# Arash-san/YinYang-Game-AlphaZero

Measured on AMD Instinct MI355X. Metric: self-play positions/sec (+ MCTS node-expansions/sec) at 800 sims, 8x8 board, higher is better.
Workload: dtype f16x3; 1 GPU; 8x8 board, 800 sims/move, 4096 concurrent games per GPU, frozen random-init 128x10 net (seed 0), copied boards, reference_quirks=False, staggered start plies; tree_arithmetic=f32 PUCT + u64 bitboards, nn_dtype=f16x3, evaluation_reuse=False, parallelism=episode-sharded x1, lanes_per_gpu=2, hipgraph=True

## Files before the change

include/yy_engine.h:

```cpp
#ifndef YY_ENGINE_H
#define YY_ENGINE_H

#include <stdint.h>

#ifdef __cplusplus
extern "C" {
#endif

#define YY_OK 0
#define YY_E_INVALID (-1)
#define YY_E_UNSUPPORTED (-2)
#define YY_E_NOMEM (-3)
#define YY_E_HIP (-4)
#define YY_E_STATE (-5)
#define YY_E_ARENA (-6)

#define YY_FLAG_ROWCOL 1u
#define YY_FLAG_ALIASED 2u
#define YY_FLAG_REUSE_PASS_VALUE 4u

#define YY_FLAG_REUSE_TRANSPOSITIONS 8u
#define YY_FLAG_KEEP_EVALUATIONS 16u

typedef void *yy_stream_t;

const char *yy_last_error(void);
int yy_version(void);


int yy_rules_valid_mask(const int8_t *boards, const int8_t *players, int G, int R, int C,
                        uint32_t flags, uint8_t *out_mask, yy_stream_t stream);

int yy_rules_step(int8_t *boards, int8_t *players, const int32_t *actions, int G, int R, int C,
                  uint32_t flags, uint8_t *placed, yy_stream_t stream);

int yy_rules_game_ended(const int8_t *boards, const int8_t *players, int G, int R, int C,
                        uint32_t flags, double *out, int32_t *counts, yy_stream_t stream);

int yy_encode_planes(const int8_t *boards, int G, int R, int C, float *out, yy_stream_t stream);

int yy_rules_mask_terminal_bb(const uint64_t *black, const uint64_t *white, int G, int R, int C,
                              uint32_t flags, uint64_t *mask_p1, uint64_t *mask_m1,
                              int8_t *result, yy_stream_t stream);

int yy_pack_boards(const int8_t *boards, int G, int R, int C, uint64_t *black, uint64_t *white,
                   yy_stream_t stream);
int yy_unpack_boards(const uint64_t *black, const uint64_t *white, int G, int R, int C,
                     int8_t *boards, yy_stream_t stream);


typedef struct yy_mcts_config {
    int32_t G;
    int32_t R, C;
    int32_t max_sims;
    float cpuct;
    uint32_t flags;
    int64_t edges_per_game;
    int64_t nodes_per_game;
} yy_mcts_config;

typedef struct yy_mcts yy_mcts;

int yy_mcts_create(const yy_mcts_config *cfg, yy_mcts **out);
int yy_mcts_destroy(yy_mcts *ctx);
int yy_mcts_memory_bytes(const yy_mcts *ctx, uint64_t *out);

int yy_mcts_begin(yy_mcts *ctx, const int8_t *boards, const int8_t *root_players,
                  const uint8_t *active, float *planes_out, yy_stream_t stream);

int yy_mcts_expand_root(yy_mcts *ctx, const float *policy, const double *noise, double eps,
                        yy_stream_t stream);

int yy_mcts_select(yy_mcts *ctx, float *planes_out, uint8_t *needs_eval, yy_stream_t stream);

int yy_mcts_expand_backup(yy_mcts *ctx, const float *policy, const float *value,
                          yy_stream_t stream);

int yy_mcts_step(yy_mcts *ctx, const float *policy, const float *value, float *planes_out,
                 uint8_t *needs_eval, yy_stream_t stream);

int yy_mcts_root_counts(yy_mcts *ctx, int32_t *counts, float *child_w, float *child_p,
                        yy_stream_t stream);

int yy_mcts_root_policy(yy_mcts *ctx, int temperature_is_zero, double *pi, yy_stream_t stream);

int yy_mcts_root_stats(yy_mcts *ctx, int32_t *visits, double *value_sum, yy_stream_t stream);

int yy_mcts_get_boards(yy_mcts *ctx, int8_t *boards, yy_stream_t stream);

int yy_mcts_status(yy_mcts *ctx, int32_t *n_overflow, uint64_t *counters);
int yy_mcts_reset_counters(yy_mcts *ctx, yy_stream_t stream);
int yy_book_insert(const uint64_t *keys, int n, int R, int C, uint32_t *meta, uint64_t *table_keys, int64_t cap,
                   int32_t *slot_of, yy_stream_t stream);
int yy_mcts_set_book(yy_mcts *ctx, const uint32_t *meta, const uint64_t *keys, const float *value, const float *policy,
                     int64_t cap, int max_stones);
int yy_mcts_cache_clear(yy_mcts *ctx, yy_stream_t stream);

int yy_nn_bias_act_bf16(void *x, const float *bias, const void *residual, int64_t rows, int C,
                        int relu, yy_stream_t stream);

int yy_nn_tower_bf16(const float *planes, const void *weights, const float *bias, void *out, int G,
                     int R, int C, int channels, int n_layers, yy_stream_t stream);

int yy_nn_tower_heads_bf16(const float *planes, const void *weights, const float *bias,
                           void *out_heads, int G, int R, int C, int channels, int n_layers,
                           yy_stream_t stream);

int yy_nn_tower_f32(const float *planes, const void *weights, const float *bias, float *out, int G,
                    int R, int C, int channels, int n_layers, yy_stream_t stream);

int yy_nn_head_finish_bf16(const void *h, int G, int A, int H, const float *w2, const float *b2,
                           float *policy, float *value, yy_stream_t stream);

int yy_nn_tower_f16x3_regs(const float *planes, const void *weights, const void *head_w, const float *bias,
                           float *out, float *out_heads, const int32_t *rows, const int32_t *n_rows, int G,
                           int R, int C, int channels, int n_layers, int weight_exp, int head_exp,
                           int act_exp, yy_stream_t stream);

int yy_nn_tower_g(const float *planes, const void *weights, const void *head_w, const float *bias, const float *head_bias,
                  float *out, float *out_heads, const int32_t *rows, const int32_t *n_rows, int G, int R, int C,
                  int channels, int n_layers, int weight_exp, int head_exp, int act_exp, int nb, int boards, int gate_lo,
                  int gate_hi, yy_stream_t stream);
int yy_nn_tower_g_forms(int channels, int *nb_out);

int yy_nn_fc_heads_f16x3(const float *feats, const void *wpk, const float *bias, const int32_t *jobs, int n_jobs,
                         float *logits, float *hidden, const int32_t *n_rows, int G, int K, int A, int H,
                         int weight_exp, int act_exp, yy_stream_t stream);

int yy_nn_head_finish_f32(const float *logits, const float *hidden, int G, int A, int H, const float *w2,
                          const float *b2, const int32_t *rows, const int32_t *n_rows, float *policy,
                          float *value, yy_stream_t stream);

int yy_compact_rows(const uint8_t *flags, int G, int32_t *rows, int32_t *n, yy_stream_t stream);

int yy_selfplay_root_noise(uint64_t seed, const int64_t *game_id, const int32_t *ply, const uint8_t *draw,
                           const uint8_t *mask, int G, int A, double alpha, double *noise, yy_stream_t stream);

int yy_selfplay_sample_actions(uint64_t seed, const int64_t *game_id, const int32_t *ply,
                               const uint8_t *searching, const double *pi, const uint8_t *mask, int G, int A,
                               int temperature_threshold, int32_t *action, yy_stream_t stream);

#ifdef __cplusplus
}
#endif
#endif
```

yinyang-game-alphazero_amd/_lib.py:

```python
import ctypes as C
import os
import subprocess

_HERE = os.path.dirname(os.path.abspath(__file__))
CSRC = os.path.join(_HERE, "csrc")
SO = os.path.join(CSRC, "libyy_hip.so")
HEADER = os.path.normpath(os.path.join(_HERE, "..", "include", "yy_engine.h"))

YY_OK = 0
YY_E_ARENA = -6
FLAG_ROWCOL = 1
FLAG_ALIASED = 2
FLAG_REUSE_PASS_VALUE = 4
FLAG_REUSE_TRANSPOSITIONS = 8
FLAG_KEEP_EVALUATIONS = 16

HIPCC_FLAGS = ["--offload-arch=gfx950", "-O3", "-std=c++17", "-fPIC", "-shared",
               "-ffp-contract=off", "-fno-fast-math", "-Wall", "-Wno-unused-function"]


class YYError(RuntimeError):
    def __init__(self, code, msg):
        super().__init__(f"libyy_hip: status {code}: {msg}")
        self.code = code


class MctsConfig(C.Structure):
    _fields_ = [("G", C.c_int32), ("R", C.c_int32), ("C", C.c_int32), ("max_sims", C.c_int32),
                ("cpuct", C.c_float), ("flags", C.c_uint32), ("edges_per_game", C.c_int64),
                ("nodes_per_game", C.c_int64)]


def build(force=False, verbose=False):
    srcs = [os.path.join(CSRC, f) for f in ("yy_engine.hip", "yy_tower.hip", "yy_towerq.hip", "yy_tower_f32.hip", "yy_tower_h3r.hip",
                                            "yy_tower_g.hip", "yy_fc_heads.hip", "yy_selfplay.hip", "yy_bitboard.h")] + [HEADER]
    if not force and os.path.exists(SO) and all(os.path.getmtime(SO) >= os.path.getmtime(s) for s in srcs):
        return SO
    hipcc = os.environ.get("HIPCC", "/opt/rocm/bin/hipcc")
    tmp = f"{SO}.{os.getpid()}.tmp"
    cmd = [hipcc] + HIPCC_FLAGS + ["-o", tmp] + [s for s in srcs if s.endswith(".hip")]
    if verbose:
        print(" ".join(cmd).replace(tmp, SO))
    try:
        subprocess.check_call(cmd)
        os.replace(tmp, SO)
    finally:
        if os.path.exists(tmp):
            os.remove(tmp)
    return SO


_LIB = None
_vp = C.c_void_p
_SIGS = {
    "yy_rules_valid_mask": [_vp, _vp, C.c_int, C.c_int, C.c_int, C.c_uint32, _vp, _vp],
    "yy_rules_step": [_vp, _vp, _vp, C.c_int, C.c_int, C.c_int, C.c_uint32, _vp, _vp],
    "yy_rules_game_ended": [_vp, _vp, C.c_int, C.c_int, C.c_int, C.c_uint32, _vp, _vp, _vp],
    "yy_encode_planes": [_vp, C.c_int, C.c_int, C.c_int, _vp, _vp],
    "yy_rules_mask_terminal_bb": [_vp, _vp, C.c_int, C.c_int, C.c_int, C.c_uint32, _vp, _vp, _vp, _vp],
    "yy_pack_boards": [_vp, C.c_int, C.c_int, C.c_int, _vp, _vp, _vp],
    "yy_unpack_boards": [_vp, _vp, C.c_int, C.c_int, C.c_int, _vp, _vp],
    "yy_mcts_create": [C.POINTER(MctsConfig), C.POINTER(_vp)],
    "yy_mcts_destroy": [_vp],
    "yy_mcts_memory_bytes": [_vp, C.POINTER(C.c_uint64)],
    "yy_mcts_begin": [_vp, _vp, _vp, _vp, _vp, _vp],
    "yy_mcts_expand_root": [_vp, _vp, _vp, C.c_double, _vp],
    "yy_mcts_select": [_vp, _vp, _vp, _vp],
    "yy_mcts_expand_backup": [_vp, _vp, _vp, _vp],
    "yy_mcts_step": [_vp, _vp, _vp, _vp, _vp, _vp],
    "yy_mcts_root_counts": [_vp, _vp, _vp, _vp, _vp],
    "yy_mcts_root_policy": [_vp, C.c_int, _vp, _vp],
    "yy_mcts_root_stats": [_vp, _vp, _vp, _vp],
    "yy_mcts_get_boards": [_vp, _vp, _vp],
    "yy_mcts_status": [_vp, C.POINTER(C.c_int32), C.POINTER(C.c_uint64)],
    "yy_mcts_reset_counters": [_vp, _vp],
    "yy_mcts_cache_clear": [_vp, _vp],
    "yy_book_insert": [_vp, C.c_int, C.c_int, C.c_int, _vp, _vp, C.c_int64, _vp, _vp],
    "yy_mcts_set_book": [_vp, _vp, _vp, _vp, _vp, C.c_int64, C.c_int],
    "yy_nn_bias_act_bf16": [_vp, _vp, _vp, C.c_int64, C.c_int, C.c_int, _vp],
    "yy_nn_tower_bf16": [_vp, _vp, _vp, _vp, C.c_int, C.c_int, C.c_int, C.c_int, C.c_int, _vp],
    "yy_nn_tower_heads_bf16": [_vp, _vp, _vp, _vp, C.c_int, C.c_int, C.c_int, C.c_int, C.c_int, _vp],
    "yy_nn_head_finish_bf16": [_vp, C.c_int, C.c_int, C.c_int, _vp, _vp, _vp, _vp, _vp],
    "yy_nn_tower_f32": [_vp, _vp, _vp, _vp, C.c_int, C.c_int, C.c_int, C.c_int, C.c_int, _vp],
    "yy_nn_head_finish_f32": [_vp, _vp, C.c_int, C.c_int, C.c_int, _vp, _vp, _vp, _vp, _vp, _vp, _vp],
    "yy_compact_rows": [_vp, C.c_int, _vp, _vp, _vp],
    "yy_nn_tower_f16x3_regs": [_vp, _vp, _vp, _vp, _vp, _vp, _vp, _vp, C.c_int, C.c_int, C.c_int, C.c_int, C.c_int, C.c_int, C.c_int,
                               C.c_int, _vp],
    "yy_nn_tower_g_forms": [C.c_int, C.POINTER(C.c_int)],
    "yy_nn_tower_g": [_vp, _vp, _vp, _vp, _vp, _vp, _vp, _vp, _vp, C.c_int, C.c_int, C.c_int, C.c_int, C.c_int, C.c_int, C.c_int,
                      C.c_int, C.c_int, C.c_int, C.c_int, C.c_int, _vp],
    "yy_nn_fc_heads_f16x3": [_vp, _vp, _vp, _vp, C.c_int, _vp, _vp, _vp, C.c_int, C.c_int, C.c_int, C.c_int, C.c_int, C.c_int, _vp],
    "yy_selfplay_root_noise": [C.c_uint64, _vp, _vp, _vp, _vp, C.c_int, C.c_int, C.c_double, _vp, _vp],
    "yy_selfplay_sample_actions": [C.c_uint64, _vp, _vp, _vp, _vp, _vp, C.c_int, C.c_int, C.c_int, _vp, _vp],
    "yy_version": [],
}


def exported_symbols():
    return sorted(list(_SIGS) + ["yy_last_error"])


def lib():
    global _LIB
    if _LIB is None:
        if not os.path.exists(SO):
            raise YYError(-100, f"{SO} is missing: run __graft_entry__.build() (hipcc --offload-arch=gfx950); "
                                "there is no CPU fallback for the product path")
        L = C.CDLL(SO)
        for name, args in _SIGS.items():
            fn = getattr(L, name)
            fn.argtypes = args
            fn.restype = C.c_int
        L.yy_last_error.restype = C.c_char_p
        L.yy_last_error.argtypes = []
        _LIB = L
    return _LIB


def check(status):
    if status != YY_OK:
        raise YYError(status, lib().yy_last_error().decode())
    return status
```

yinyang-game-alphazero_amd/csrc/yy_tower_g.hip:

```cpp
#include <hip/hip_runtime.h>
#include <math.h>
#include <stdint.h>

#include <type_traits>

#include "../../include/yy_engine.h"

typedef __attribute__((ext_vector_type(8))) _Float16 f16x8;
typedef __attribute__((ext_vector_type(2))) _Float16 f16x2;
typedef __attribute__((ext_vector_type(4))) float f32x4;
typedef __attribute__((ext_vector_type(2))) float f32x2;
typedef __attribute__((ext_vector_type(4))) unsigned int u32x4;
typedef __attribute__((ext_vector_type(2))) unsigned int u32x2;

extern "C" int yy_tower_set_err(int code, const char *msg);

namespace tg {

__device__ __forceinline__ float relu_keep_nan(float v) { return __builtin_isnan(v) ? v : fmaxf(v, 0.0f); }

template <int NW_, int NB_, int D_> struct Geo {
    static constexpr int NW = NW_, NB = NB_, D = D_, CH = 32 * NW_, NCOL = 16 * NB_;
    static constexpr int RS = (NW_ >= 3) ? 288 : 160;
    static constexpr int ZERO_OFF = NCOL * RS;
    static constexpr int PART_BYTES = ZERO_OFF + 512;
    static constexpr int RES_OFF = 2 * PART_BYTES;
    static constexpr int LDS_BYTES = RES_OFF + NW_ * 2 * NB_ * 1024;
    static constexpr int CHUNK_BYTES = NW_ * 4096;
    static_assert(9 % D_ == 0, "ring position = tap % D");
    static_assert(ZERO_OFF % 256 == 0 && PART_BYTES % 256 == 0, "zero rows / parts keep the bank phase");
    static_assert(PART_BYTES + 256 < 65536 && LDS_BYTES <= 163840, "LDS layout");
};

__device__ __forceinline__ void split_pair(const f32x2 a, uint32_t &hi, uint32_t &lo) {
    const f16x2 h = __builtin_convertvector(a, f16x2);
    const f32x2 r = a - __builtin_convertvector(h, f32x2);
    const f16x2 l = __builtin_convertvector(r, f16x2);
    hi = __builtin_bit_cast(uint32_t, h);
    lo = __builtin_bit_cast(uint32_t, l);
}
__device__ __forceinline__ f32x2 join_pair(const uint32_t hi, const uint32_t lo) {
    const f32x2 h = __builtin_convertvector(__builtin_bit_cast(f16x2, hi), f32x2);
    const f32x2 l = __builtin_convertvector(__builtin_bit_cast(f16x2, lo), f32x2);
    return h + l;
}

struct WChunk {
    f16x8 h[2], l[2];
};
__device__ __forceinline__ void load_w(WChunk &w, const unsigned char *wbase, uint32_t voff) {
    const u32x4 *p = (const u32x4 *)(wbase + voff);
    w.h[0] = __builtin_bit_cast(f16x8, p[0]);
    w.l[0] = __builtin_bit_cast(f16x8, p[64]);
    w.h[1] = __builtin_bit_cast(f16x8, p[128]);
    w.l[1] = __builtin_bit_cast(f16x8, p[192]);
}

template <class GEO> struct LaneGeo {
    uint32_t rowbase[GEO::NB], okmask[GEO::NB];
};
template <class GEO> __device__ __forceinline__ void make_lane_geo(LaneGeo<GEO> &g, int lane, int R, int C, int n_valid_cols) {
    const int n = lane & 15, kg = lane >> 4, cells = R * C;
#pragma unroll
    for (int nb = 0; nb < GEO::NB; nb++) {
        const int col = nb * 16 + n;
        const int cell = col % cells;
        const int y = cell / C, x = cell - y * C;
        g.rowbase[nb] = (uint32_t)(col * GEO::RS + kg * 16);
        uint32_t m = 0;
#pragma unroll
        for (int tap = 0; tap < 9; tap++) {
            const int sy = y + tap / 3 - 1, sx = x + tap % 3 - 1;
            if (((unsigned)sy < (unsigned)R) && ((unsigned)sx < (unsigned)C)) m |= 1u << tap;
        }
        g.okmask[nb] = (col < n_valid_cols) ? m : 0u;
    }
}
template <class GEO, int TAP>
__device__ __forceinline__ uint32_t tap_addr(int nb, int crs, const LaneGeo<GEO> &g) {
    const int shift = (TAP / 3 - 1) * crs + (TAP % 3 - 1) * GEO::RS;
    const uint32_t a = g.rowbase[nb] + (uint32_t)shift;
    return (g.okmask[nb] & (1u << TAP)) ? a : ((a & 255u) | (uint32_t)GEO::ZERO_OFF);
}

template <int NB> struct XWin {
    static constexpr int P = NB;
    f16x8 h[P], l[P];
};
template <class GEO> __device__ __forceinline__ void load_x1(XWin<GEO::NB> &f, int slot, const unsigned char *lds, uint32_t cb) {
    f.h[slot] = __builtin_bit_cast(f16x8, *(const u32x4 *)(lds + cb));
    f.l[slot] = __builtin_bit_cast(f16x8, *(const u32x4 *)(lds + cb + GEO::PART_BYTES));
}
template <bool ZERO>
__device__ __forceinline__ void mma6(f32x4 (&acc1)[2], f32x4 (&acc2)[2], const WChunk &w, const f16x8 xh, const f16x8 xl) {
    const f32x4 z = {0.f, 0.f, 0.f, 0.f};
#pragma unroll
    for (int mb = 0; mb < 2; mb++) {
        const f32x4 a = __builtin_amdgcn_mfma_f32_16x16x32_f16(w.l[mb], xh, ZERO ? z : acc2[mb], 0, 0, 0);
        acc1[mb] = __builtin_amdgcn_mfma_f32_16x16x32_f16(w.h[mb], xh, ZERO ? z : acc1[mb], 0, 0, 0);
        acc2[mb] = __builtin_amdgcn_mfma_f32_16x16x32_f16(w.h[mb], xl, a, 0, 0, 0);
    }
}

template <class GEO, int J, bool ZERO>
__device__ __forceinline__ void run_chunk(f32x4 (&acc1)[GEO::NB][2], f32x4 (&acc2)[GEO::NB][2], const WChunk &w, XWin<GEO::NB> &X,
                                          const unsigned char *lds_cur, const unsigned char *lds_next, int crs, const LaneGeo<GEO> &geo) {
    constexpr int NB = GEO::NB, P = XWin<NB>::P;
#pragma unroll
    for (int nb = 0; nb < NB; nb++) {
        mma6<ZERO>(acc1[nb], acc2[nb], w, X.h[nb % P], X.l[nb % P]);
        if (nb + P < NB) load_x1<GEO>(X, nb % P, lds_cur, tap_addr<GEO, J>(nb + P, crs, geo));
        else load_x1<GEO>(X, nb % P, lds_next, tap_addr<GEO, (J + 1) % 9>(nb + P - NB, crs, geo));
        __builtin_amdgcn_sched_group_barrier(0x008, 6, 0);
        __builtin_amdgcn_sched_group_barrier(0x100, 2, 0);
    }
}

template <class GEO, bool STEM>
__device__ __forceinline__ void run_layer(f32x4 (&acc1)[GEO::NB][2], f32x4 (&acc2)[GEO::NB][2], WChunk (&W)[GEO::D], const unsigned char *lds,
                                          const unsigned char *weights, uint32_t voff, int &chunk, int n_tower, int crs,
                                          const LaneGeo<GEO> &geo) {
    constexpr int KQ = STEM ? 1 : GEO::NW, NB = GEO::NB, D = GEO::D, P = XWin<NB>::P;
    XWin<NB> X;
#pragma unroll
    for (int nb = 0; nb < P; nb++) load_x1<GEO>(X, nb, lds, tap_addr<GEO, 0>(nb, crs, geo));
    auto step = [&](auto jt, auto zt, const unsigned char *lds_cur, const unsigned char *lds_next) {
        constexpr int J = decltype(jt)::value, S = J % D;
        run_chunk<GEO, J, decltype(zt)::value>(acc1, acc2, W[S], X, lds_cur, lds_next, crs, geo);
        load_w(W[S], weights + (size_t)min(chunk + D, n_tower - 1) * GEO::CHUNK_BYTES, voff);
        __builtin_amdgcn_sched_group_barrier(0x020, 4, 0);
        __builtin_amdgcn_sched_barrier(0);
        chunk++;
    };
    auto taps = [&](auto zt, const unsigned char *cur, const unsigned char *nxt) {
        step(std::integral_constant<int, 0>{}, zt, cur, cur);
        step(std::integral_constant<int, 1>{}, std::false_type{}, cur, cur);
        step(std::integral_constant<int, 2>{}, std::false_type{}, cur, cur);
        step(std::integral_constant<int, 3>{}, std::false_type{}, cur, cur);
        step(std::integral_constant<int, 4>{}, std::false_type{}, cur, cur);
        step(std::integral_constant<int, 5>{}, std::false_type{}, cur, cur);
        step(std::integral_constant<int, 6>{}, std::false_type{}, cur, cur);
        step(std::integral_constant<int, 7>{}, std::false_type{}, cur, cur);
        step(std::integral_constant<int, 8>{}, std::false_type{}, cur, nxt);
    };
    taps(std::true_type{}, lds, lds + 64);
#pragma unroll 1
    for (int kq = 1; kq < KQ; kq++) taps(std::false_type{}, lds + kq * 64, lds + (kq + 1) * 64);
}

template <int NW_, int NB_, int D_>
__global__ void __launch_bounds__(64 * NW_, 1)
k_tower_g(const float *__restrict__ planes, const unsigned char *__restrict__ weights, const unsigned char *__restrict__ head_w,
          const float *__restrict__ bias, const float *__restrict__ head_bias, float *__restrict__ out, float *__restrict__ out_heads,
          const int *__restrict__ rows, const int *__restrict__ n_rows, int G, int R, int C, int TB, int n_layers, float in_scale,
          float acc_scale, float head_scale, float out_scale, int gate_lo, int gate_hi) {
    using GEO = Geo<NW_, NB_, D_>;
    constexpr int NW = GEO::NW, NB = GEO::NB, D = GEO::D, CH = GEO::CH, RS = GEO::RS, NT = 64 * NW_;
    __shared__ __attribute__((aligned(256))) unsigned char lds[GEO::LDS_BYTES];
    const int n_live = n_rows ? min(*n_rows, G) : G;
    if (n_live <= gate_lo || n_live > gate_hi) return;
    const int g0 = blockIdx.x * TB;
    if (g0 >= n_live) return;
    const int lane = threadIdx.x & 63;
    const int wave = __builtin_amdgcn_readfirstlane(threadIdx.x >> 6);
    const int cells = R * C, ncol = TB * cells;
    const int n_tower = 9 + 9 * NW * (n_layers - 1), crs = C * RS;

    const uint32_t voff = (uint32_t)(wave * 4096 + lane * 16);
    WChunk W[D];
#pragma unroll
    for (int j = 0; j < D; j++) load_w(W[j], weights + (size_t)min(j, n_tower - 1) * GEO::CHUNK_BYTES, voff);

    for (int t = threadIdx.x; t < 128; t += NT)
        ((u32x2 *)(lds + GEO::ZERO_OFF + (t >> 6) * GEO::PART_BYTES))[t & 63] = (u32x2){0u, 0u};
    for (int col = threadIdx.x; col < GEO::NCOL; col += NT) {
        const int gb = g0 + col / cells, cell = col % cells;
        const bool live = col < ncol && gb < n_live;
        const int src = live ? (rows ? rows[gb] : gb) : 0;
        float p[6];
#pragma unroll
        for (int k = 0; k < 5; k++) p[k] = live ? planes[((size_t)src * 5 + k) * cells + cell] * in_scale : 0.0f;
        p[5] = 0.0f;
        uint32_t hi[3], lo[3];
#pragma unroll
        for (int k = 0; k < 3; k++) split_pair((f32x2){p[2 * k], p[2 * k + 1]}, hi[k], lo[k]);
        const u32x4 z = {0u, 0u, 0u, 0u};
        *(u32x4 *)(lds + col * RS) = (u32x4){hi[0], hi[1], hi[2], 0u};
        *(u32x4 *)(lds + GEO::PART_BYTES + col * RS) = (u32x4){lo[0], lo[1], lo[2], 0u};
#pragma unroll
        for (int q = 1; q < 4; q++) {
            *(u32x4 *)(lds + col * RS + 16 * q) = z;
            *(u32x4 *)(lds + GEO::PART_BYTES + col * RS + 16 * q) = z;
        }
    }

    LaneGeo<GEO> geo;
    make_lane_geo<GEO>(geo, lane, R, C, ncol);
    const int n16 = lane & 15, kg = lane >> 4;
    unsigned char *res_lds = lds + GEO::RES_OFF + (wave * 2 * NB) * 1024 + lane * 16;
    int chunk = 0;
    auto epilogue = [&](const int L, f32x4 (&acc1)[NB][2], f32x4 (&acc2)[NB][2], auto conv2_tag, auto keep_tag) {
        constexpr bool CONV2 = decltype(conv2_tag)::value, KEEP = decltype(keep_tag)::value;
        const float *bl = bias + L * CH + wave * 32;
        float sb[32];
#pragma unroll
        for (int k = 0; k < 32; k++) {
            sb[k] = bl[k];
            asm volatile("" : "+s"(sb[k]));
        }
        f32x4 bq[2];
#pragma unroll
        for (int mb = 0; mb < 2; mb++)
#pragma unroll
            for (int i = 0; i < 4; i++)
                bq[mb][i] = kg == 0 ? sb[mb * 16 + i] : kg == 1 ? sb[mb * 16 + 4 + i] : kg == 2 ? sb[mb * 16 + 8 + i] : sb[mb * 16 + 12 + i];
#pragma unroll
        for (int nb = 0; nb < NB; nb++) {
            const uint32_t rowoff = (uint32_t)((nb * 16 + n16) * RS);
#pragma unroll
            for (int mb = 0; mb < 2; mb++) {
                f32x4 v;
#pragma unroll
                for (int i = 0; i < 4; i++) v[i] = __builtin_fmaf(acc1[nb][mb][i] + acc2[nb][mb][i], acc_scale, bq[mb][i]);
                if (CONV2) v += *(const f32x4 *)(res_lds + (mb * NB + nb) * 1024);
#pragma unroll
                for (int i = 0; i < 4; i++) v[i] = relu_keep_nan(v[i]);
                if (KEEP) *(f32x4 *)(res_lds + (mb * NB + nb) * 1024) = v;
                uint32_t h01, l01, h23, l23;
                split_pair((f32x2){v[0], v[1]}, h01, l01);
                split_pair((f32x2){v[2], v[3]}, h23, l23);
                const uint32_t co2 = (uint32_t)((wave * 32 + mb * 16 + kg * 4) * 2);
                *(u32x2 *)(lds + rowoff + co2) = (u32x2){h01, h23};
                *(u32x2 *)(lds + GEO::PART_BYTES + rowoff + co2) = (u32x2){l01, l23};
            }
        }
    };
    {
        f32x4 acc1[NB][2], acc2[NB][2];
        __syncthreads();
        run_layer<GEO, true>(acc1, acc2, W, lds, weights, voff, chunk, n_tower, crs, geo);
        __syncthreads();
        epilogue(0, acc1, acc2, std::false_type{}, std::true_type{});
    }
    for (int L = 1; L < n_layers; L++) {
        f32x4 acc1[NB][2], acc2[NB][2];
        __syncthreads();
        run_layer<GEO, false>(acc1, acc2, W, lds, weights, voff, chunk, n_tower, crs, geo);
        __syncthreads();
        if ((L & 1) == 0) epilogue(L, acc1, acc2, std::true_type{}, std::true_type{});
        else epilogue(L, acc1, acc2, std::false_type{}, std::false_type{});
    }
    __syncthreads();
    if (out_heads) {
        int lane2 = lane;
        asm volatile("" : "+v"(lane2));
        const int n16 = lane2 & 15, kg = lane2 >> 4;
        for (int hm = wave; hm < 4; hm += NW) {
            const int head = hm >> 1, mb = hm & 1;
            f16x8 wh[NW], wl[NW];
#pragma unroll
            for (int kq = 0; kq < NW; kq++) {
                const unsigned char *p = head_w + ((size_t)(hm * NW + kq) * 2) * 1024 + lane2 * 16;
                wh[kq] = __builtin_bit_cast(f16x8, *(const u32x4 *)p);
                wl[kq] = __builtin_bit_cast(f16x8, *(const u32x4 *)(p + 1024));
            }
            const float *hb = head_bias + head * 32 + mb * 16;
            float sb[16];
#pragma unroll
            for (int k = 0; k < 16; k++) {
                sb[k] = hb[k];
                asm volatile("" : "+s"(sb[k]));
            }
            f32x4 b;
#pragma unroll
            for (int i = 0; i < 4; i++) b[i] = kg == 0 ? sb[i] : kg == 1 ? sb[4 + i] : kg == 2 ? sb[8 + i] : sb[12 + i];
#pragma unroll
            for (int nb = 0; nb < NB; nb++) {
                const uint32_t xb = (uint32_t)((nb * 16 + n16) * RS + kg * 16);
                f32x4 h1 = {0.f, 0.f, 0.f, 0.f}, h2 = {0.f, 0.f, 0.f, 0.f};
#pragma unroll
                for (int kq = 0; kq < NW; kq++) {
                    const f16x8 xh = __builtin_bit_cast(f16x8, *(const u32x4 *)(lds + xb + kq * 64));
                    const f16x8 xl = __builtin_bit_cast(f16x8, *(const u32x4 *)(lds + xb + GEO::PART_BYTES + kq * 64));
                    const f32x4 a = __builtin_amdgcn_mfma_f32_16x16x32_f16(wl[kq], xh, h2, 0, 0, 0);
                    h1 = __builtin_amdgcn_mfma_f32_16x16x32_f16(wh[kq], xh, h1, 0, 0, 0);
                    h2 = __builtin_amdgcn_mfma_f32_16x16x32_f16(wh[kq], xl, a, 0, 0, 0);
                }
                const int col = nb * 16 + n16;
                const int gb = g0 + col / cells, cell = col % cells;
                if (col < ncol && gb < n_live) {
                    float *o = out_heads + (((size_t)gb * 2 + head) * 32 + mb * 16 + kg * 4) * cells + cell;
#pragma unroll
                    for (int i = 0; i < 4; i++) o[i * cells] = relu_keep_nan(__builtin_fmaf(h1[i] + h2[i], head_scale, b[i]));
                }
            }
        }
        return;
    }
    for (int p = threadIdx.x; p < ncol * (CH / 4); p += NT) {
        const int col = p / (CH / 4), ch4 = p % (CH / 4);
        if (g0 + col / cells < n_live) {
            const u32x2 ph = *(const u32x2 *)(lds + col * RS + ch4 * 8);
            const u32x2 pl = *(const u32x2 *)(lds + GEO::PART_BYTES + col * RS + ch4 * 8);
            const f32x2 v01 = join_pair(ph.x, pl.x), v23 = join_pair(ph.y, pl.y);
            *(f32x4 *)(out + ((size_t)g0 * cells + col) * CH + ch4 * 4) = (f32x4){v01.x, v01.y, v23.x, v23.y} * out_scale;
        }
    }
}

}

namespace {

struct TgArgs {
    const float *planes;
    const void *weights, *head_w;
    const float *bias, *head_bias;
    float *out, *out_heads;
    const int *rows, *n_rows;
    int G, R, C, TB, n_layers;
    float sc[4];
    int gate_lo, gate_hi;
    hipStream_t s;
};

template <int NW, int NB, int D> int launch_tg(const TgArgs &a) {
    tg::k_tower_g<NW, NB, D><<<dim3((a.G + a.TB - 1) / a.TB), dim3(64 * NW), 0, a.s>>>(
        a.planes, (const unsigned char *)a.weights, (const unsigned char *)a.head_w, a.bias, a.head_bias, a.out, a.out_heads, a.rows,
        a.n_rows, a.G, a.R, a.C, a.TB, a.n_layers, a.sc[0], a.sc[1], a.sc[2], a.sc[3], a.gate_lo, a.gate_hi);
    if (hipGetLastError() != hipSuccess) return yy_tower_set_err(YY_E_HIP, "yy_nn_tower_g: launch failed");
    return YY_OK;
}

int dispatch_tg(int nw, int nb, const TgArgs &a) {
    if (nw == 4) {
        switch (nb) {
        case 4: return launch_tg<4, 4, 9>(a);
        case 5: return launch_tg<4, 5, 9>(a);
        case 6: return launch_tg<4, 6, 9>(a);
        case 7: return launch_tg<4, 7, 9>(a);
        case 8: return launch_tg<4, 8, 9>(a);
        case 9: return launch_tg<4, 9, 9>(a);
        }
    } else if (nb == 4 || nb == 9) {
        if (nw == 1) return nb == 4 ? launch_tg<1, 4, 9>(a) : launch_tg<1, 9, 3>(a);
        if (nw == 2) return nb == 4 ? launch_tg<2, 4, 9>(a) : launch_tg<2, 9, 3>(a);
        if (nw == 3) return nb == 4 ? launch_tg<3, 4, 9>(a) : launch_tg<3, 9, 3>(a);
    }
    return yy_tower_set_err(YY_E_UNSUPPORTED, "yy_nn_tower_g: no kernel form for this (channels, column blocks)");
}

}

extern "C" int yy_nn_tower_g_forms(int channels, int *nb_out) {
    if (channels == 128) {
        for (int i = 0; i < 6; i++) nb_out[i] = 4 + i;
        return 6;
    }
    if (channels == 32 || channels == 64 || channels == 96) {
        nb_out[0] = 4;
        nb_out[1] = 9;
        return 2;
    }
    return 0;
}

extern "C" int yy_nn_tower_g(const float *planes, const void *weights, const void *head_w, const float *bias, const float *head_bias,
                             float *out, float *out_heads, const int32_t *rows, const int32_t *n_rows, int G, int R, int C,
                             int channels, int n_layers, int weight_exp, int head_exp, int act_exp, int nb, int boards, int gate_lo,
                             int gate_hi, yy_stream_t s) {
    if (G == 0) return YY_OK;
    if (!planes || !weights || !bias || (!out && !out_heads) || (out_heads && (!head_w || !head_bias)) || G < 0 || (rows && !n_rows))
        return yy_tower_set_err(YY_E_INVALID, "yy_nn_tower_g: bad argument");
    if (R < 1 || C < 1 || R * C > 144 || channels < 32 || channels > 128 || (channels & 31) || n_layers < 1 || n_layers > 21 ||
        (n_layers & 1) == 0)
        return yy_tower_set_err(YY_E_UNSUPPORTED,
                                "yy_nn_tower_g: needs boards of at most 144 cells, 32/64/96/128 channels, at most 10 residual blocks");
    if (boards < 1 || nb < 1 || boards * R * C > 16 * nb) return yy_tower_set_err(YY_E_INVALID, "yy_nn_tower_g: boards * cells > 16 * nb");
    TgArgs a = {planes, weights, head_w, bias, head_bias, out, out_heads, rows, n_rows, G, R, C, boards, n_layers,
                {ldexpf(1.0f, act_exp), ldexpf(1.0f, -weight_exp), ldexpf(1.0f, -(head_exp + act_exp)), ldexpf(1.0f, -act_exp)},
                gate_lo, gate_hi, (hipStream_t)s};
    return dispatch_tg(channels / 32, nb, a);
}
```

yinyang-game-alphazero_amd/engine.py:

```python
import ctypes as ct

import torch

from . import _lib
from ._lib import FLAG_ALIASED, FLAG_REUSE_PASS_VALUE, FLAG_KEEP_EVALUATIONS, FLAG_REUSE_TRANSPOSITIONS, FLAG_ROWCOL, MctsConfig, check, lib


def _stream():
    return ct.c_void_p(torch.cuda.current_stream().cuda_stream)


def _p(t):
    return None if t is None else ct.c_void_p(t.data_ptr())


def _need(t, dtype, shape=None, name="tensor"):
    if not isinstance(t, torch.Tensor) or not t.is_cuda:
        raise _lib.YYError(-1, f"{name}: expected a ROCm device tensor (the hot path has no CPU fallback)")
    if t.dtype != dtype or not t.is_contiguous():
        raise _lib.YYError(-1, f"{name}: expected contiguous {dtype}, got {t.dtype} contiguous={t.is_contiguous()}")
    if shape is not None and tuple(t.shape) != tuple(shape):
        raise _lib.YYError(-1, f"{name}: expected shape {tuple(shape)}, got {tuple(t.shape)}")
    return t

# ... 3 lines not shown


def valid_mask(boards, players, rowcol=False):
    G, R, Cc = boards.shape
    _need(boards, torch.int8, name="boards")
    _need(players, torch.int8, (G,), "players")
    out = torch.empty((G, R * Cc), dtype=torch.uint8, device=boards.device)
    with torch.cuda.device(boards.device):
        check(lib().yy_rules_valid_mask(_p(boards), _p(players), G, R, Cc, _flags(rowcol), _p(out), _stream()))
    return out


def step_(boards, players, actions, rowcol=False):
    G, R, Cc = boards.shape
    _need(boards, torch.int8, name="boards")
    _need(players, torch.int8, (G,), "players")
    _need(actions, torch.int32, (G,), "actions")
    placed = torch.empty(G, dtype=torch.uint8, device=boards.device)
    with torch.cuda.device(boards.device):
        check(lib().yy_rules_step(_p(boards), _p(players), _p(actions), G, R, Cc, _flags(rowcol), _p(placed), _stream()))
    return placed


def game_ended(boards, players, rowcol=False, with_counts=False):
    G, R, Cc = boards.shape
    _need(boards, torch.int8, name="boards")
    _need(players, torch.int8, (G,), "players")
    out = torch.empty(G, dtype=torch.float64, device=boards.device)
    counts = torch.empty((G, 2), dtype=torch.int32, device=boards.device) if with_counts else None
    with torch.cuda.device(boards.device):
        check(lib().yy_rules_game_ended(_p(boards), _p(players), G, R, Cc, _flags(rowcol), _p(out), _p(counts), _stream()))
    return (out, counts) if with_counts else out


def encode_planes(boards, out=None):
    G, R, Cc = boards.shape
    _need(boards, torch.int8, name="boards")
    if out is None:
        out = torch.empty((G, 5, R, Cc), dtype=torch.float32, device=boards.device)
    _need(out, torch.float32, (G, 5, R, Cc), "out")
    with torch.cuda.device(boards.device):
        check(lib().yy_encode_planes(_p(boards), G, R, Cc, _p(out), _stream()))
    return out


def pack_boards(boards):
    G, R, Cc = boards.shape
    _need(boards, torch.int8, name="boards")
    nw = (R * Cc + 63) // 64
    black = torch.empty((nw, G), dtype=torch.int64, device=boards.device)
    white = torch.empty((nw, G), dtype=torch.int64, device=boards.device)
    with torch.cuda.device(boards.device):
        check(lib().yy_pack_boards(_p(boards), G, R, Cc, _p(black), _p(white), _stream()))
    return black, white


def unpack_boards(black, white, R, Cc):
    nw, G = black.shape
    _need(black, torch.int64, name="black")
    _need(white, torch.int64, (nw, G), "white")
    boards = torch.empty((G, R, Cc), dtype=torch.int8, device=black.device)
    with torch.cuda.device(black.device):
        check(lib().yy_unpack_boards(_p(black), _p(white), G, R, Cc, _p(boards), _stream()))
    return boards


def mask_terminal_bb(black, white, R, Cc, rowcol=False, out=None):
    nw, G = black.shape
    _need(black, torch.int64, name="black")
    _need(white, torch.int64, (nw, G), "white")
    if out is None:
        out = (torch.empty_like(black), torch.empty_like(black),
               torch.empty(G, dtype=torch.int8, device=black.device))
    m1, m2, res = out
    with torch.cuda.device(black.device):
        check(lib().yy_rules_mask_terminal_bb(_p(black), _p(white), G, R, Cc, _flags(rowcol), _p(m1), _p(m2), _p(res), _stream()))
    return m1, m2, res


def bias_act_(x, bias, residual=None, relu=True):
    if x.dim() != 4 or not x.is_contiguous(memory_format=torch.channels_last) or x.dtype != torch.bfloat16 or not x.is_cuda:
        raise _lib.YYError(-1, "bias_act_: expected a channels-last bf16 device tensor [N,C,H,W]")
    N, Cc, H, W = x.shape
    if bias.dtype != torch.float32 or bias.numel() != Cc or not bias.is_cuda:
        raise _lib.YYError(-1, "bias_act_: bias must be float32 [C] on the device")
    if residual is not None and (residual.shape != x.shape or residual.dtype != x.dtype
                                 or not residual.is_contiguous(memory_format=torch.channels_last)):
        raise _lib.YYError(-1, "bias_act_: residual must match x (channels-last bf16)")
    with torch.cuda.device(x.device):
        check(lib().yy_nn_bias_act_bf16(_p(x), _p(bias), _p(residual), N * H * W, Cc, int(bool(relu)), _stream()))
    return x


def tower_forward(planes, weights, bias, n_layers):
    G, _, R, Cc = planes.shape
    _need(planes, torch.float32, (G, 5, R, Cc), "planes")
    n_chunks = 9 + 18 * (n_layers - 1)
    _need(weights, torch.int16, (n_chunks, 8192), "tower weights")
    _need(bias, torch.float32, (n_layers, 128), "tower bias")
    out = torch.empty((G, R, Cc, 128), dtype=torch.bfloat16, device=planes.device)
    with torch.cuda.device(planes.device):
        check(lib().yy_nn_tower_bf16(_p(planes), _p(weights), _p(bias), _p(out), G, R, Cc, 128, n_layers, _stream()))
    return out.permute(0, 3, 1, 2)


def tower_forward_f32(planes, weights, bias, n_layers):
    G = planes.shape[0]
    _need(planes, torch.float32, (G, 5, 8, 8), "planes")
    _need(weights, torch.float32, (9 + 36 * (n_layers - 1), 4096), "f32 tower weights")
    _need(bias, torch.float32, (n_layers, 128), "tower bias")
    out = torch.empty((G, 8, 8, 128), dtype=torch.float32, device=planes.device)
    with torch.cuda.device(planes.device):
        check(lib().yy_nn_tower_f32(_p(planes), _p(weights), _p(bias), _p(out), G, 8, 8, 128, n_layers, _stream()))
    return out.permute(0, 3, 1, 2)


def tower_heads_forward_h3r(planes, weights, head_w, bias, n_layers, exps, rows=None, n_rows=None, out=None):
    G, _, R, Cc = planes.shape
    _need(planes, torch.float32, (G, 5, R, Cc), "planes")
    _need(weights, torch.int16, (9 + 36 * (n_layers - 1), 8192), "wave-major split-f16 tower weights")
    _need(head_w, torch.int16, (2, 8192), "wave-major split-f16 head weights")
    _need(bias, torch.float32, (n_layers + 1, 128), "tower+heads bias")
    if rows is not None:
        _need(rows, torch.int32, (G,), "rows")
        _need(n_rows, torch.int32, (1,), "n_rows")
    if out is None:
        out = torch.empty((G, 2, 32 * R * Cc), dtype=torch.float32, device=planes.device)
    _need(out, torch.float32, (G, 2, 32 * R * Cc), "out")
    with torch.cuda.device(planes.device):
        check(lib().yy_nn_tower_f16x3_regs(_p(planes), _p(weights), _p(head_w), _p(bias), None, _p(out), _p(rows), _p(n_rows), G, R, Cc,
                                           128, n_layers, int(exps[0]), int(exps[1]), int(exps[2]), _stream()))
    return out


def tower_forward_h3r(planes, weights, bias, n_layers, exps):
    G, _, R, Cc = planes.shape
    _need(planes, torch.float32, (G, 5, R, Cc), "planes")
    _need(weights, torch.int16, (9 + 36 * (n_layers - 1), 8192), "wave-major split-f16 tower weights")
    _need(bias, torch.float32, (n_layers, 128), "tower bias")
    out = torch.empty((G, R, Cc, 128), dtype=torch.float32, device=planes.device)
    with torch.cuda.device(planes.device):
        check(lib().yy_nn_tower_f16x3_regs(_p(planes), _p(weights), None, _p(bias), _p(out), None, None, None, G, R, Cc, 128, n_layers,
                                           int(exps[0]), 0, int(exps[2]), _stream()))
    return out.permute(0, 3, 1, 2)


def tower_g_available(channels):
    buf = (ct.c_int * 8)()
    n = lib().yy_nn_tower_g_forms(int(channels), buf)
    return [int(buf[i]) for i in range(n)]


def tower_g(planes, weights, bias, n_layers, exps, nb, boards, head_w=None, head_bias=None, rows=None, n_rows=None, out=None,
            gate=(-1, 0x7FFFFFFF)):
    G, _, R, Cc = planes.shape
    _need(planes, torch.float32, (G, 5, R, Cc), "planes")
    ch = bias.shape[1]
    nw = ch // 32
    _need(weights, torch.int16, (9 + 9 * nw * (n_layers - 1), ch * 64), "split-f16 tower weights (pack_tower_g)")
    _need(bias, torch.float32, (n_layers, ch), "tower bias")
    if rows is not None:
        _need(rows, torch.int32, (G,), "rows")
        _need(n_rows, torch.int32, (1,), "n_rows")
    heads = head_w is not None
    if heads:
        _need(head_w, torch.int16, (4 * nw * 2 * 512,), "split-f16 head weights (pack_heads_g)")
        _need(head_bias, torch.float32, (64,), "head bias")
        if out is None:
            out = torch.empty((G, 2, 32 * R * Cc), dtype=torch.float32, device=planes.device)
        _need(out, torch.float32, (G, 2, 32 * R * Cc), "out")
    else:
        out = torch.empty((G, R, Cc, ch), dtype=torch.float32, device=planes.device)
    with torch.cuda.device(planes.device):
        check(lib().yy_nn_tower_g(_p(planes), _p(weights), _p(head_w), _p(bias), _p(head_bias), None if heads else _p(out),
                                  _p(out) if heads else None, _p(rows), _p(n_rows), G, R, Cc, ch, n_layers, int(exps[0]), int(exps[1]),
                                  int(exps[2]), int(nb), int(boards), int(gate[0]), int(gate[1]), _stream()))
    return out if heads else out.permute(0, 3, 1, 2)


def fc_heads(feats, wpk, bias, jobs, A, H, exps, n_rows=None, logits=None, hidden=None):
    G, two, K = feats.shape
    _need(feats, torch.float32, (G, 2, K), "feats")
    _need(jobs, torch.int32, (jobs.shape[0], 4), "jobs")
    ksteps = ((K + 127) // 128) * 4
    _need(wpk, torch.int16, (jobs.shape[0] * ksteps * 4096,), "fc head weights (pack_fc_heads)")
    _need(bias, torch.float32, (A + H,), "fc head bias")
    if n_rows is not None:
        _need(n_rows, torch.int32, (1,), "n_rows")
    if logits is None:
        logits = torch.empty((G, A), dtype=torch.float32, device=feats.device)
        hidden = torch.empty((G, H), dtype=torch.float32, device=feats.device)
    _need(logits, torch.float32, (G, A), "logits")
    _need(hidden, torch.float32, (G, H), "hidden")
    with torch.cuda.device(feats.device):
        check(lib().yy_nn_fc_heads_f16x3(_p(feats), _p(wpk), _p(bias), _p(jobs), jobs.shape[0], _p(logits), _p(hidden), _p(n_rows), G, K,
                                         A, H, int(exps[0]), int(exps[1]), _stream()))
    return logits, hidden


def head_finish_f32(logits, hidden, w2, b2, rows=None, n_rows=None, policy=None, value=None):
    G, A = logits.shape
    _need(logits, torch.float32, name="logits")
    _need(hidden, torch.float32, (G, hidden.shape[1]), "hidden")
    _need(w2, torch.float32, (hidden.shape[1],), "w2")
    _need(b2, torch.float32, (1,), "b2")
    if rows is not None:
        _need(rows, torch.int32, (G,), "rows")
        _need(n_rows, torch.int32, (1,), "n_rows")
    if policy is None:
        policy = torch.zeros((G, A), dtype=torch.float32, device=logits.device)
        value = torch.zeros(G, dtype=torch.float32, device=logits.device)
    _need(policy, torch.float32, (G, A), "policy")
    _need(value, torch.float32, (G,), "value")
    with torch.cuda.device(logits.device):
        check(lib().yy_nn_head_finish_f32(_p(logits), _p(hidden), G, A, hidden.shape[1], _p(w2), _p(b2), _p(rows), _p(n_rows),
                                          _p(policy), _p(value), _stream()))
    return policy, value


def compact_rows(flags, rows=None, n=None):
    G = flags.shape[0]
    _need(flags, torch.uint8, (G,), "flags")
    if rows is None:
        rows = torch.zeros(G, dtype=torch.int32, device=flags.device)
        n = torch.zeros(1, dtype=torch.int32, device=flags.device)
    _need(rows, torch.int32, (G,), "rows")
    _need(n, torch.int32, (1,), "n")
    with torch.cuda.device(flags.device):
        check(lib().yy_compact_rows(_p(flags), G, _p(rows), _p(n), _stream()))
    return rows, n


def tower_heads_forward(planes, weights, bias, n_layers):
    G, _, R, Cc = planes.shape
    _need(planes, torch.float32, (G, 5, R, Cc), "planes")
    n_chunks = 9 + 18 * (n_layers - 1) + 1
    _need(weights, torch.int16, (n_chunks, 8192), "tower+heads weights")
    _need(bias, torch.float32, (n_layers + 1, 128), "tower+heads bias")
    out = torch.empty((G, 2, 32 * R * Cc), dtype=torch.bfloat16, device=planes.device)
    with torch.cuda.device(planes.device):
        check(lib().yy_nn_tower_heads_bf16(_p(planes), _p(weights), _p(bias), _p(out), G, R, Cc, 128, n_layers, _stream()))
    return out


def head_finish(h, A, w2, b2):
    G, W = h.shape
    _need(h, torch.bfloat16, name="h")
    _need(w2, torch.float32, (W - A,), "w2")
    _need(b2, torch.float32, (1,), "b2")
    policy = torch.empty((G, A), dtype=torch.float32, device=h.device)
    value = torch.empty(G, dtype=torch.float32, device=h.device)
    with torch.cuda.device(h.device):
        check(lib().yy_nn_head_finish_bf16(_p(h), G, A, W - A, _p(w2), _p(b2), _p(policy), _p(value), _stream()))
    return policy, value


def root_noise(seed, game_id, ply, draw, mask, alpha):
    G, A = mask.shape
    _need(game_id, torch.int64, (G,), "game_id")
    _need(ply, torch.int32, (G,), "ply")
    _need(draw, torch.uint8, (G,), "draw")
    _need(mask, torch.uint8, (G, A), "mask")
    out = torch.empty((G, A), dtype=torch.float64, device=mask.device)
    with torch.cuda.device(mask.device):
        check(lib().yy_selfplay_root_noise(ct.c_uint64(int(seed) & (2 ** 64 - 1)), _p(game_id), _p(ply), _p(draw), _p(mask), G, A,
                                           float(alpha), _p(out), _stream()))
    return out


def sample_actions(seed, game_id, ply, searching, pi, mask, temperature_threshold):
    G, A = mask.shape
    _need(game_id, torch.int64, (G,), "game_id")
    _need(ply, torch.int32, (G,), "ply")
    _need(searching, torch.uint8, (G,), "searching")
    _need(pi, torch.float64, (G, A), "pi")
    _need(mask, torch.uint8, (G, A), "mask")
    out = torch.empty(G, dtype=torch.int32, device=mask.device)
    with torch.cuda.device(mask.device):
        check(lib().yy_selfplay_sample_actions(ct.c_uint64(int(seed) & (2 ** 64 - 1)), _p(game_id), _p(ply), _p(searching), _p(pi),
                                               _p(mask), G, A, int(temperature_threshold), _p(out), _stream()))
    return out


class OpeningBook:

    def __init__(self, R, C, evaluator, max_stones, rowcol=False, batch=4096, device=None, max_positions=8_000_000):
        dev = torch.device("cuda", torch.cuda.current_device()) if device is None else torch.device(device)
        self.R, self.C, self.A, self.max_stones = int(R), int(C), int(R) * int(C), int(max_stones)
        nw = (self.A + 63) // 64
        boards = torch.zeros((1, R, C), dtype=torch.int8, device=dev)
        player, keys, states = 1, [], []
        for _ in range(self.max_stones):
            players = torch.full((boards.shape[0],), player, dtype=torch.int8, device=dev)
            vm = valid_mask(boards, players, rowcol)
            n_children = int(vm.sum())
            if n_children == 0:
                break
            if n_children > 8 * max_positions:
                self.max_stones = len(keys)
                break
            bi, a = vm.nonzero(as_tuple=True)
            child = boards.reshape(-1, self.A)[bi]
            child[torch.arange(bi.numel(), device=dev), a] = player
            black, white = pack_boards(child.view(-1, R, C))
            key = torch.cat([black.t(), white.t()], dim=1).contiguous()
            uniq, inv = torch.unique(key, dim=0, return_inverse=True)
            first = torch.zeros(uniq.shape[0], dtype=torch.int64, device=dev)
            first[inv] = torch.arange(key.shape[0], device=dev)
            if sum(k.shape[0] for k in keys) + uniq.shape[0] > max_positions:
                self.max_stones = len(keys)
                break
            boards = child[first].view(-1, R, C).contiguous()
            keys.append(uniq)
            states.append(boards)
            player = -player
        if not keys:
            raise _lib.YYError(-1, "OpeningBook: nothing to store (max_stones < 1 or max_positions too small)")
        self.keys = torch.cat(keys).contiguous()
        boards = torch.cat(states)
        self.n = int(self.keys.shape[0])
        pol = torch.empty((self.n, self.A), dtype=torch.float32, device=dev)
        val = torch.empty(self.n, dtype=torch.float32, device=dev)
        for lo in range(0, self.n, batch):
            p, v = evaluator(encode_planes(boards[lo:lo + batch].contiguous()))
            pol[lo:lo + batch], val[lo:lo + batch] = p, v
        self.cap = 64
        while self.cap < 6 * self.n:
            self.cap *= 2
        self.meta = torch.zeros(self.cap, dtype=torch.int32, device=dev)
# ... 169 lines not shown
```

Before: 1561 positions/s.

## Add row-aligned board layout to tower kernel and skip off-board tap MFMAs

Adds a row-blocked column layout to the conv tower kernel. When boards*C equals 16 and nb equals R, each 16-column block holds one board row across the tile's boards, so padding taps above the first row and below the last row are known at compile time. The MFMAs and LDS loads for those taps are skipped statically, which cuts matrix work for the 3x3 taps. The column-to-board/cell mapping changes throughout staging, the heads and output writes, which adds integer index work and new template instantiations; the old column-major layout stays available behind a flag.

```diff
diff --git a/include/yy_engine.h b/include/yy_engine.h
--- a/include/yy_engine.h
+++ b/include/yy_engine.h
@@ -120,7 +120,7 @@
 int yy_nn_tower_g(const float *planes, const void *weights, const void *head_w, const float *bias, const float *head_bias,
                   float *out, float *out_heads, const int32_t *rows, const int32_t *n_rows, int G, int R, int C,
                   int channels, int n_layers, int weight_exp, int head_exp, int act_exp, int nb, int boards, int gate_lo,
-                  int gate_hi, yy_stream_t stream);
+                  int gate_hi, int layout, yy_stream_t stream);
 int yy_nn_tower_g_forms(int channels, int *nb_out);
 
 int yy_nn_fc_heads_f16x3(const float *feats, const void *wpk, const float *bias, const int32_t *jobs, int n_jobs,
diff --git a/yinyang-game-alphazero_amd/_lib.py b/yinyang-game-alphazero_amd/_lib.py
--- a/yinyang-game-alphazero_amd/_lib.py
+++ b/yinyang-game-alphazero_amd/_lib.py
@@ -88,7 +88,7 @@
                                C.c_int, _vp],
     "yy_nn_tower_g_forms": [C.c_int, C.POINTER(C.c_int)],
     "yy_nn_tower_g": [_vp, _vp, _vp, _vp, _vp, _vp, _vp, _vp, _vp, C.c_int, C.c_int, C.c_int, C.c_int, C.c_int, C.c_int, C.c_int,
-                      C.c_int, C.c_int, C.c_int, C.c_int, C.c_int, _vp],
+                      C.c_int, C.c_int, C.c_int, C.c_int, C.c_int, C.c_int, _vp],
     "yy_nn_fc_heads_f16x3": [_vp, _vp, _vp, _vp, C.c_int, _vp, _vp, _vp, C.c_int, C.c_int, C.c_int, C.c_int, C.c_int, C.c_int, _vp],
     "yy_selfplay_root_noise": [C.c_uint64, _vp, _vp, _vp, _vp, C.c_int, C.c_int, C.c_double, _vp, _vp],
     "yy_selfplay_sample_actions": [C.c_uint64, _vp, _vp, _vp, _vp, _vp, C.c_int, C.c_int, C.c_int, _vp, _vp],
diff --git a/yinyang-game-alphazero_amd/csrc/yy_tower_g.hip b/yinyang-game-alphazero_amd/csrc/yy_tower_g.hip
--- a/yinyang-game-alphazero_amd/csrc/yy_tower_g.hip
+++ b/yinyang-game-alphazero_amd/csrc/yy_tower_g.hip
@@ -19,8 +19,9 @@
 
 __device__ __forceinline__ float relu_keep_nan(float v) { return __builtin_isnan(v) ? v : fmaxf(v, 0.0f); }
 
-template <int NW_, int NB_, int D_> struct Geo {
+template <int NW_, int NB_, int D_, bool RB_> struct Geo {
     static constexpr int NW = NW_, NB = NB_, D = D_, CH = 32 * NW_, NCOL = 16 * NB_;
+    static constexpr bool RB = RB_;
     static constexpr int RS = (NW_ >= 3) ? 288 : 160;
     static constexpr int ZERO_OFF = NCOL * RS;
     static constexpr int PART_BYTES = ZERO_OFF + 512;
@@ -56,15 +57,27 @@
     w.l[1] = __builtin_bit_cast(f16x8, p[192]);
 }
 
+template <class GEO> __device__ __forceinline__ void col_board_cell(int col, int C, int cells, int &board, int &cell) {
+    if constexpr (GEO::RB) {
+        const int n = col & 15;
+        board = n / C;
+        cell = (col >> 4) * C + (n - board * C);
+    } else {
+        board = col / cells;
+        cell = col - board * cells;
+    }
+}
+
 template <class GEO> struct LaneGeo {
     uint32_t rowbase[GEO::NB], okmask[GEO::NB];
 };
-template <class GEO> __device__ __forceinline__ void make_lane_geo(LaneGeo<GEO> &g, int lane, int R, int C, int n_valid_cols) {
+template <class GEO> __device__ __forceinline__ void make_lane_geo(LaneGeo<GEO> &g, int lane, int R, int C, int TB) {
     const int n = lane & 15, kg = lane >> 4, cells = R * C;
 #pragma unroll
     for (int nb = 0; nb < GEO::NB; nb++) {
         const int col = nb * 16 + n;
-        const int cell = col % cells;
+        int board, cell;
+        col_board_cell<GEO>(col, C, cells, board, cell);
         const int y = cell / C, x = cell - y * C;
         g.rowbase[nb] = (uint32_t)(col * GEO::RS + kg * 16);
         uint32_t m = 0;
@@ -73,7 +86,7 @@
             const int sy = y + tap / 3 - 1, sx = x + tap % 3 - 1;
             if (((unsigned)sy < (unsigned)R) && ((unsigned)sx < (unsigned)C)) m |= 1u << tap;
         }
-        g.okmask[nb] = (col < n_valid_cols) ? m : 0u;
+        g.okmask[nb] = (board < TB) ? m : 0u;
     }
 }
 template <class GEO, int TAP>
@@ -81,6 +94,10 @@
     const int shift = (TAP / 3 - 1) * crs + (TAP % 3 - 1) * GEO::RS;
     const uint32_t a = g.rowbase[nb] + (uint32_t)shift;
     return (g.okmask[nb] & (1u << TAP)) ? a : ((a & 255u) | (uint32_t)GEO::ZERO_OFF);
+}
+
+template <class GEO> constexpr bool off_board(int tap, int nb) {
+    return GEO::RB && ((nb == 0 && tap < 3) || (nb == GEO::NB - 1 && tap >= 6));
 }
 
 template <int NB> struct XWin {
@@ -106,13 +123,15 @@
 __device__ __forceinline__ void run_chunk(f32x4 (&acc1)[GEO::NB][2], f32x4 (&acc2)[GEO::NB][2], const WChunk &w, XWin<GEO::NB> &X,
                                           const unsigned char *lds_cur, const unsigned char *lds_next, int crs, const LaneGeo<GEO> &geo) {
     constexpr int NB = GEO::NB, P = XWin<NB>::P;
+    static_assert(!GEO::RB || P == NB, "the row-aligned skips assume the full window");
 #pragma unroll
     for (int nb = 0; nb < NB; nb++) {
-        mma6<ZERO>(acc1[nb], acc2[nb], w, X.h[nb % P], X.l[nb % P]);
+        const bool mma = !off_board<GEO>(J, nb), ld = nb + P < NB || !off_board<GEO>((J + 1) % 9, nb + P - NB);
+        if (mma) mma6<ZERO>(acc1[nb], acc2[nb], w, X.h[nb % P], X.l[nb % P]);
         if (nb + P < NB) load_x1<GEO>(X, nb % P, lds_cur, tap_addr<GEO, J>(nb + P, crs, geo));
-        else load_x1<GEO>(X, nb % P, lds_next, tap_addr<GEO, (J + 1) % 9>(nb + P - NB, crs, geo));
-        __builtin_amdgcn_sched_group_barrier(0x008, 6, 0);
-        __builtin_amdgcn_sched_group_barrier(0x100, 2, 0);
+        else if (ld) load_x1<GEO>(X, nb % P, lds_next, tap_addr<GEO, (J + 1) % 9>(nb + P - NB, crs, geo));
+        if (mma) __builtin_amdgcn_sched_group_barrier(0x008, 6, 0);
+        if (ld) __builtin_amdgcn_sched_group_barrier(0x100, 2, 0);
     }
 }
 
@@ -123,7 +142,12 @@
     constexpr int KQ = STEM ? 1 : GEO::NW, NB = GEO::NB, D = GEO::D, P = XWin<NB>::P;
     XWin<NB> X;
 #pragma unroll
-    for (int nb = 0; nb < P; nb++) load_x1<GEO>(X, nb, lds, tap_addr<GEO, 0>(nb, crs, geo));
+    for (int nb = 0; nb < P; nb++)
+        if (!off_board<GEO>(0, nb)) load_x1<GEO>(X, nb, lds, tap_addr<GEO, 0>(nb, crs, geo));
+    if constexpr (GEO::RB) {
+#pragma unroll
+        for (int mb = 0; mb < 2; mb++) acc1[0][mb] = acc2[0][mb] = (f32x4){0.f, 0.f, 0.f, 0.f};
+    }
     auto step = [&](auto jt, auto zt, const unsigned char *lds_cur, const unsigned char *lds_next) {
         constexpr int J = decltype(jt)::value, S = J % D;
         run_chunk<GEO, J, decltype(zt)::value>(acc1, acc2, W[S], X, lds_cur, lds_next, crs, geo);
@@ -148,13 +172,13 @@
     for (int kq = 1; kq < KQ; kq++) taps(std::false_type{}, lds + kq * 64, lds + (kq + 1) * 64);
 }
 
-template <int NW_, int NB_, int D_>
+template <int NW_, int NB_, int D_, bool RB_>
 __global__ void __launch_bounds__(64 * NW_, 1)
 k_tower_g(const float *__restrict__ planes, const unsigned char *__restrict__ weights, const unsigned char *__restrict__ head_w,
           const float *__restrict__ bias, const float *__restrict__ head_bias, float *__restrict__ out, float *__restrict__ out_heads,
           const int *__restrict__ rows, const int *__restrict__ n_rows, int G, int R, int C, int TB, int n_layers, float in_scale,
           float acc_scale, float head_scale, float out_scale, int gate_lo, int gate_hi) {
-    using GEO = Geo<NW_, NB_, D_>;
+    using GEO = Geo<NW_, NB_, D_, RB_>;
     constexpr int NW = GEO::NW, NB = GEO::NB, D = GEO::D, CH = GEO::CH, RS = GEO::RS, NT = 64 * NW_;
     __shared__ __attribute__((aligned(256))) unsigned char lds[GEO::LDS_BYTES];
     const int n_live = n_rows ? min(*n_rows, G) : G;
@@ -164,7 +188,7 @@
     const int lane = threadIdx.x & 63;
     const int wave = __builtin_amdgcn_readfirstlane(threadIdx.x >> 6);
     const int cells = R * C, ncol = TB * cells;
-    const int n_tower = 9 + 9 * NW * (n_layers - 1), crs = C * RS;
+    const int n_tower = 9 + 9 * NW * (n_layers - 1), crs = (GEO::RB ? 16 : C) * RS;
 
     const uint32_t voff = (uint32_t)(wave * 4096 + lane * 16);
     WChunk W[D];
@@ -174,8 +198,10 @@
     for (int t = threadIdx.x; t < 128; t += NT)
         ((u32x2 *)(lds + GEO::ZERO_OFF + (t >> 6) * GEO::PART_BYTES))[t & 63] = (u32x2){0u, 0u};
     for (int col = threadIdx.x; col < GEO::NCOL; col += NT) {
-        const int gb = g0 + col / cells, cell = col % cells;
-        const bool live = col < ncol && gb < n_live;
+        int b, cell;
+        col_board_cell<GEO>(col, C, cells, b, cell);
+        const int gb = g0 + b;
+        const bool live = b < TB && gb < n_live;
         const int src = live ? (rows ? rows[gb] : gb) : 0;
         float p[6];
 #pragma unroll
@@ -195,7 +221,7 @@
     }
 
     LaneGeo<GEO> geo;
-    make_lane_geo<GEO>(geo, lane, R, C, ncol);
+    make_lane_geo<GEO>(geo, lane, R, C, TB);
     const int n16 = lane & 15, kg = lane >> 4;
     unsigned char *res_lds = lds + GEO::RES_OFF + (wave * 2 * NB) * 1024 + lane * 16;
     int chunk = 0;
@@ -286,9 +312,10 @@
                     h1 = __builtin_amdgcn_mfma_f32_16x16x32_f16(wh[kq], xh, h1, 0, 0, 0);
                     h2 = __builtin_amdgcn_mfma_f32_16x16x32_f16(wh[kq], xl, a, 0, 0, 0);
                 }
-                const int col = nb * 16 + n16;
-                const int gb = g0 + col / cells, cell = col % cells;
-                if (col < ncol && gb < n_live) {
+                int bd, cell;
+                col_board_cell<GEO>(nb * 16 + n16, C, cells, bd, cell);
+                const int gb = g0 + bd;
+                if (bd < TB && gb < n_live) {
                     float *o = out_heads + (((size_t)gb * 2 + head) * 32 + mb * 16 + kg * 4) * cells + cell;
 #pragma unroll
                     for (int i = 0; i < 4; i++) o[i * cells] = relu_keep_nan(__builtin_fmaf(h1[i] + h2[i], head_scale, b[i]));
@@ -299,11 +326,13 @@
     }
     for (int p = threadIdx.x; p < ncol * (CH / 4); p += NT) {
         const int col = p / (CH / 4), ch4 = p % (CH / 4);
-        if (g0 + col / cells < n_live) {
+        int b, cell;
+        col_board_cell<GEO>(col, C, cells, b, cell);
+        if (b < TB && g0 + b < n_live) {
             const u32x2 ph = *(const u32x2 *)(lds + col * RS + ch4 * 8);
             const u32x2 pl = *(const u32x2 *)(lds + GEO::PART_BYTES + col * RS + ch4 * 8);
             const f32x2 v01 = join_pair(ph.x, pl.x), v23 = join_pair(ph.y, pl.y);
-            *(f32x4 *)(out + ((size_t)g0 * cells + col) * CH + ch4 * 4) = (f32x4){v01.x, v01.y, v23.x, v23.y} * out_scale;
+            *(f32x4 *)(out + ((size_t)(g0 + b) * cells + cell) * CH + ch4 * 4) = (f32x4){v01.x, v01.y, v23.x, v23.y} * out_scale;
         }
     }
 }
@@ -324,16 +353,19 @@
     hipStream_t s;
 };
 
-template <int NW, int NB, int D> int launch_tg(const TgArgs &a) {
-    tg::k_tower_g<NW, NB, D><<<dim3((a.G + a.TB - 1) / a.TB), dim3(64 * NW), 0, a.s>>>(
+template <int NW, int NB, int D, bool RB = false> int launch_tg(const TgArgs &a) {
+    tg::k_tower_g<NW, NB, D, RB><<<dim3((a.G + a.TB - 1) / a.TB), dim3(64 * NW), 0, a.s>>>(
         a.planes, (const unsigned char *)a.weights, (const unsigned char *)a.head_w, a.bias, a.head_bias, a.out, a.out_heads, a.rows,
         a.n_rows, a.G, a.R, a.C, a.TB, a.n_layers, a.sc[0], a.sc[1], a.sc[2], a.sc[3], a.gate_lo, a.gate_hi);
     if (hipGetLastError() != hipSuccess) return yy_tower_set_err(YY_E_HIP, "yy_nn_tower_g: launch failed");
     return YY_OK;
 }
 
-int dispatch_tg(int nw, int nb, const TgArgs &a) {
+int dispatch_tg(int nw, int nb, bool columns, const TgArgs &a) {
+    const bool rb = !columns && a.TB * a.C == 16 && nb == a.R;
     if (nw == 4) {
+        if (rb && nb == 8) return launch_tg<4, 8, 9, true>(a);
+        if (rb && nb == 4) return launch_tg<4, 4, 9, true>(a);
         switch (nb) {
         case 4: return launch_tg<4, 4, 9>(a);
         case 5: return launch_tg<4, 5, 9>(a);
@@ -368,17 +400,17 @@
 extern "C" int yy_nn_tower_g(const float *planes, const void *weights, const void *head_w, const float *bias, const float *head_bias,
                              float *out, float *out_heads, const int32_t *rows, const int32_t *n_rows, int G, int R, int C,
                              int channels, int n_layers, int weight_exp, int head_exp, int act_exp, int nb, int boards, int gate_lo,
-                             int gate_hi, yy_stream_t s) {
+                             int gate_hi, int layout, yy_stream_t s) {
     if (G == 0) return YY_OK;
     if (!planes || !weights || !bias || (!out && !out_heads) || (out_heads && (!head_w || !head_bias)) || G < 0 || (rows && !n_rows))
         return yy_tower_set_err(YY_E_INVALID, "yy_nn_tower_g: bad argument");
     if (R < 1 || C < 1 || R * C > 144 || channels < 32 || channels > 128 || (channels & 31) || n_layers < 1 || n_layers > 21 ||
-        (n_layers & 1) == 0)
+        (n_layers & 1) == 0 || layout < 0 || layout > 1)
         return yy_tower_set_err(YY_E_UNSUPPORTED,
                                 "yy_nn_tower_g: needs boards of at most 144 cells, 32/64/96/128 channels, at most 10 residual blocks");
     if (boards < 1 || nb < 1 || boards * R * C > 16 * nb) return yy_tower_set_err(YY_E_INVALID, "yy_nn_tower_g: boards * cells > 16 * nb");
     TgArgs a = {planes, weights, head_w, bias, head_bias, out, out_heads, rows, n_rows, G, R, C, boards, n_layers,
                 {ldexpf(1.0f, act_exp), ldexpf(1.0f, -weight_exp), ldexpf(1.0f, -(head_exp + act_exp)), ldexpf(1.0f, -act_exp)},
                 gate_lo, gate_hi, (hipStream_t)s};
-    return dispatch_tg(channels / 32, nb, a);
-}
+    return dispatch_tg(channels / 32, nb, layout == 1, a);
+}
diff --git a/yinyang-game-alphazero_amd/engine.py b/yinyang-game-alphazero_amd/engine.py
--- a/yinyang-game-alphazero_amd/engine.py
+++ b/yinyang-game-alphazero_amd/engine.py
@@ -179,7 +179,7 @@
 
 
 def tower_g(planes, weights, bias, n_layers, exps, nb, boards, head_w=None, head_bias=None, rows=None, n_rows=None, out=None,
-            gate=(-1, 0x7FFFFFFF)):
+            gate=(-1, 0x7FFFFFFF), column_layout=False):
     G, _, R, Cc = planes.shape
     _need(planes, torch.float32, (G, 5, R, Cc), "planes")
     ch = bias.shape[1]
@@ -201,7 +201,8 @@
     with torch.cuda.device(planes.device):
         check(lib().yy_nn_tower_g(_p(planes), _p(weights), _p(head_w), _p(bias), _p(head_bias), None if heads else _p(out),
                                   _p(out) if heads else None, _p(rows), _p(n_rows), G, R, Cc, ch, n_layers, int(exps[0]), int(exps[1]),
-                                  int(exps[2]), int(nb), int(boards), int(gate[0]), int(gate[1]), _stream()))
+                                  int(exps[2]), int(nb), int(boards), int(gate[0]), int(gate[1]), int(bool(column_layout)),
+                                  _stream()))
     return out if heads else out.permute(0, 3, 1, 2)
 
 
```

Measured after the change: 1682 positions/s, median of 6. 7.8% higher.
